# z430/keyword-spotting

Measured on AMD Instinct MI355X. Metric: 1s 16kHz clips/sec end-to-end (wav->label), higher is better.
Workload: dtype f32

## Files before the change

### keyword-spotting_amd/csrc/kws_dscnn.hip

```cpp
#include <type_traits>

#include "kws_internal.h"
#include "kws_mfcc_dev.h"
#include "kws_split_mfma.h"

namespace kws {
namespace {


#ifndef KWS_DSCNN_WAVES
#define KWS_DSCNN_WAVES 8
#endif
#ifndef KWS_X_DSCNN_STAMP_TID
#define KWS_X_DSCNN_STAMP_TID 0
#endif
constexpr int NW = KWS_DSCNN_WAVES;
constexpr int NT = NW * 64;
constexpr int TW = 30;

constexpr int P0 = C1_H * C1_W;
constexpr int FEAT_H = 103, FEAT_W = 14;
constexpr int OFF_Z3 = 0, OFF_Z2 = 22976, OFF_Z1 = 0, OFF_Z0 = 9152, OFF_FEAT = 18304;
constexpr int OFF_DWTAB = 38784;
constexpr int OFF_PWB = OFF_DWTAB + 2 * 768;
constexpr int OFF_POOLED = OFF_PWB + 2 * 64;
constexpr int OFF_POOLBUF = OFF_DWTAB;
constexpr int OFF_WMAX = OFF_POOLED + 64 + 8;
constexpr int LDS_FLOATS = 40960;
static_assert(OFF_WMAX + 4 * NW <= LDS_FLOATS, "LDS overflow");
static_assert(NW * 64 <= 768, "pool scratch must fit one depthwise buffer");
static_assert(OFF_FEAT + FEAT_H * FEAT_W <= OFF_Z2, "feature pad overlaps Z2");
static_assert(CH * 12 <= 2 * NT, "table staging assumes at most two elements per thread");

__device__ __forceinline__ constexpr int pidx(int c, int p, int S) { return (c >> 1) * 2 * S + 2 * p + (c & 1); }

template <int N>
struct Blk {
    static constexpr int H = 45 + 2 * N, W = 1 + 2 * N;
    static constexpr bool RING = N > 1;
    static constexpr int HI = RING ? H - 2 : H, WI = RING ? W - 2 : W;
    static constexpr int PIN = HI * WI, SIN = PIN + 2;
    static constexpr int POUT = H * W, SOUT = POUT + 2;
    static constexpr int OFF_IN = N == 1 ? OFF_Z0 : N == 2 ? OFF_Z1 : N == 3 ? OFF_Z2 : OFF_Z3;
    static constexpr int OFF_OUT = N == 1 ? OFF_Z1 : N == 2 ? OFF_Z2 : OFF_Z3;
    static constexpr int TILES = (POUT + TW - 1) / TW;
    static constexpr int BUF = (N - 1) & 1;
};

#ifndef KWS_DSCNN_KSPLIT_LEFTOVER
#define KWS_DSCNN_KSPLIT_LEFTOVER 1
#endif
template <int N>
struct Leftover {
    static constexpr bool HAS = KWS_DSCNN_KSPLIT_LEFTOVER && (N == 1 || N == 2);
    static constexpr int TILE = N == 1 ? 4 : 8;
    static constexpr int P0T = TILE * TW;
    static constexpr int NP = HAS ? Blk<N>::POUT - P0T : 1;
    static constexpr int WAVE0 = N == 1 ? 4 : 0;
    static constexpr int OFF_PART = N == 1 ? OFF_Z2 : OFF_Z0;
};
static_assert(Blk<1>::TILES == 5 && Blk<2>::TILES == 9, "the leftover tiles are the fifth of block 1 and the ninth of block 2");
static_assert(4 * CH * Leftover<1>::NP <= 38784 - OFF_Z2 && OFF_Z0 + 4 * CH * Leftover<2>::NP <= OFF_FEAT, "partial sums fit their dead planes");

constexpr int OFF_FEAT_P = OFF_Z2;
constexpr int OFF_POOLBUF_P = OFF_FEAT_P + 1456;
constexpr int STAGE_WAVES = 4;
static_assert(OFF_FEAT_P >= OFF_Z3 + Blk<3>::SOUT * CH, "the next clip's features must not overlap block 4's input");
static_assert(OFF_FEAT_P + FEAT_H * FEAT_W <= OFF_POOLBUF_P && OFF_POOLBUF_P % 4 == 0, "features and pool partials are disjoint");
static_assert(OFF_POOLBUF_P + NW * CH <= OFF_Z2 + Blk<2>::SOUT * CH && OFF_Z2 + Blk<2>::SOUT * CH <= OFF_DWTAB,
              "pool partials stay inside the Z2 plane, clear of the table buffers the next clip's block 1 rewrites");

template <bool TO_MFMA = false>
__device__ __forceinline__ float stencil3x3(float w0, float w1, float w2, float w3, float w4, float w5, float w6,
                                            float w7, float w8, float b, float up, float mid, float dn, float mask_l,
                                            float mask_r) {
    float c, to_right, to_left;
    asm("v_mul_f32 %1, %3, %13\n\t"
        "v_mul_f32 %2, %5, %13\n\t"
        "v_fma_f32 %0, %4, %13, %12\n\t"
        "v_fmac_f32 %1, %6, %14\n\t"
        "v_fmac_f32 %2, %8, %14\n\t"
        "v_fmac_f32 %0, %7, %14\n\t"
        "v_fmac_f32 %1, %9, %15\n\t"
        "v_fmac_f32 %2, %11, %15\n\t"
        "v_fmac_f32 %0, %10, %15\n\t"
        "v_fmac_f32_dpp %0, %1, %16 wave_shr:1 row_mask:0xf bank_mask:0xf bound_ctrl:1\n\t"
        "v_fmac_f32_dpp %0, %2, %17 wave_shl:1 row_mask:0xf bank_mask:0xf bound_ctrl:1"
        : "=&v"(c), "=&v"(to_right), "=&v"(to_left)
        : "v"(w0), "v"(w1), "v"(w2), "v"(w3), "v"(w4), "v"(w5), "v"(w6), "v"(w7), "v"(w8), "v"(b), "v"(up), "v"(mid),
          "v"(dn), "v"(mask_l), "v"(mask_r));
    if constexpr (TO_MFMA) asm volatile("s_nop 1" : "+v"(c));
    return c;
}
struct DwPair {
    float4 l[5];
};
template <bool TO_MFMA, int E>
__device__ __forceinline__ float stencil3x3_of_pair(const DwPair& w, float up, float mid, float dn, float mask_l, float mask_r) {
    if constexpr (E == 0)
        return stencil3x3<TO_MFMA>(w.l[0].x, w.l[0].z, w.l[1].x, w.l[1].z, w.l[2].x, w.l[2].z, w.l[3].x, w.l[3].z, w.l[4].x, w.l[4].z, up, mid, dn,
                                   mask_l, mask_r);
    else
        return stencil3x3<TO_MFMA>(w.l[0].y, w.l[0].w, w.l[1].y, w.l[1].w, w.l[2].y, w.l[2].w, w.l[3].y, w.l[3].w, w.l[4].y, w.l[4].w, up, mid, dn,
                                   mask_l, mask_r);
}
__device__ __forceinline__ float half_wave_sum_to_last_lane(float v) {
    v = dpp_shift_add<0x111, 0xf>(v);
    v = dpp_shift_add<0x112, 0xf>(v);
    v = dpp_shift_add<0x114, 0xf>(v);
    v = dpp_shift_add<0x118, 0xf>(v);
    v = dpp_shift_add<0x142, 0xa>(v);
    return v;
}

struct BlockTables {
    float d0, d1, b;
};
__device__ __forceinline__ void fetch_block_tables(const DscnnWeights& w, int n, int tid, BlockTables& r) {
    const float* src = w.dw_w + (n - 1) * CH * 12;
    r.d0 = tid < CH * 12 ? src[tid] : 0.f;
    r.d1 = NT + tid < CH * 12 ? src[NT + tid] : 0.f;
    r.b = tid < CH ? w.pw_b[(n - 1) * CH + tid] : 0.f;
}
__device__ __forceinline__ void store_block_tables(float* lds, int n, int tid, const BlockTables& r, float s_dwb = 1.f, float s_pwb = 1.f,
                                                   float s_dww = 1.f) {
    float* dwtab = lds + OFF_DWTAB + ((n - 1) & 1) * 768;
    if (tid < CH * 12) dwtab[tid] = r.d0 * ((tid % 24) >> 1 == 9 ? s_dwb : s_dww);
    if (NT + tid < CH * 12) dwtab[NT + tid] = r.d1 * (((NT + tid) % 24) >> 1 == 9 ? s_dwb : s_dww);
    if (tid < CH) lds[OFF_PWB + ((n - 1) & 1) * 64 + tid] = r.b * s_pwb;
}
struct PairCtx {
    float s_dww = 1.f;
    float s_dwb = 1.f;
    float s_pwb = 1.f;
    float inv_out = 1.f;
};
__device__ __forceinline__ void cap_units(int& ky, int& sg, int k_w, float bz) {
    sg = ky + k_w;
    const int eb = (int)((__builtin_bit_cast(uint32_t, bz) >> 23) & 0xffu) - 126;
    int limit = 100 - eb;
    limit = limit > 120 ? 120 : limit;
    if (sg > limit) {
        ky -= sg - limit;
        sg = limit;
    }
}
__device__ __forceinline__ void publish_wave_max(float* lds, int set, int wv, int lane, float mx) {
    auto step = [](float m, auto ctrl, auto row_mask) {
        return fmaxf(m, __builtin_bit_cast(float, __builtin_amdgcn_update_dpp(__builtin_bit_cast(int, m), __builtin_bit_cast(int, m), decltype(ctrl)::value,
                                                                              decltype(row_mask)::value, 0xf, false)));
    };
    mx = step(mx, std::integral_constant<int, 0x111>{}, std::integral_constant<int, 0xf>{});
    mx = step(mx, std::integral_constant<int, 0x112>{}, std::integral_constant<int, 0xf>{});
    mx = step(mx, std::integral_constant<int, 0x114>{}, std::integral_constant<int, 0xf>{});
    mx = step(mx, std::integral_constant<int, 0x118>{}, std::integral_constant<int, 0xf>{});
    mx = step(mx, std::integral_constant<int, 0x142>{}, std::integral_constant<int, 0xa>{});
    mx = step(mx, std::integral_constant<int, 0x143>{}, std::integral_constant<int, 0xc>{});
    if (lane == 63) lds[OFF_WMAX + set * NW + wv] = mx;
}
__device__ __forceinline__ float read_stage_max(const float* lds, int set0, int n_sets) {
    static_assert(NW % 4 == 0 && OFF_WMAX % 4 == 0, "the stage maxima are read as float4s");
    float m = 0.f;
    const float4* q = reinterpret_cast<const float4*>(lds + OFF_WMAX + set0 * NW);
    for (int i = 0; i < (NW / 4) * n_sets; ++i) {
        const float4 v = q[i];
        m = fmaxf(fmaxf(m, fmaxf(v.x, v.y)), fmaxf(v.z, v.w));
    }
    return m;
}

template <int NP>
struct PwRing {
    uintx4 ring[2][2][NP];
};
struct PwRegsF32 {
    float wa[2][32];
};
template <int MODE>
using PwOperands = std::conditional_t<(MODE >= 4), PwRing<(MODE == 5 ? 2 : 3)>, PwRegsF32>;
__device__ __forceinline__ void load_pointwise(const DscnnWeights& w, int n, int lane, PwRegsF32& o) {
    const float* pw = w.pw_w + (n - 1) * CH * CH + 8 * (lane >> 5) * CH + (lane & 31);
#pragma unroll
    for (int ct = 0; ct < 2; ++ct)
#pragma unroll
        for (int s = 0; s < 32; ++s) o.wa[ct][s] = pw[(16 * (s >> 3) + (s & 7)) * CH + ct * 32];
}
template <int NP>
__device__ __forceinline__ void load_afrag(const DscnnWeights& w, int n, int m, int lane, uintx4 (&f)[2][NP]) {
    const uintx4* src = reinterpret_cast<const uintx4*>(NP == 2 ? w.pw_pair : w.pw_split) + (size_t)(n - 1) * (2 * 4 * NP * 64) + lane;
#pragma unroll
    for (int ct = 0; ct < 2; ++ct)
#pragma unroll
        for (int p = 0; p < NP; ++p) f[ct][p] = src[((ct * 4 + m) * NP + p) * 64];
}
__device__ __forceinline__ void load_block_head(const DscnnWeights& w, int n, int lane, PwRegsF32& o) { load_pointwise(w, n, lane, o); }
template <int NP>
__device__ __forceinline__ void load_block_head(const DscnnWeights& w, int n, int lane, PwRing<NP>& o) { load_afrag(w, n, 0, lane, o.ring[0]); }

template <bool MFMA>
__device__ __forceinline__ void conv1_phase(const DscnnWeights& w, float* lds, int tid, const float (&a)[50]) {
    const float* featp = lds + OFF_FEAT;
    float* z0 = lds + OFF_Z0;
    if constexpr (MFMA) {
        const int lane = tid & 63, wv = tid >> 6, half = lane >> 5, col = lane & 31;
        const int ct = wv & 1;
        for (int u = wv; u < 10; u += NW) {
            const int pt = u >> 1;
            const int pos = pt * 32 + col;
            const int posc = pos < P0 ? pos : P0 - 1;
            const int oh = posc / C1_W, ow = posc % C1_W;
// ... 138 lines not shown
            __builtin_amdgcn_sched_barrier(0);
            product(5);
        }
        if (DUAL && kb + 2 < 7) {
            load_other(kb + 2);
            __builtin_amdgcn_sched_barrier(0);
        }
    }
    acc += acc2;
    occ += occ2;
    if (pos < p_hi) {
#pragma unroll
        for (int r = 0; r < 16; r += 2) {
            const int co = ct * 32 + row_of(r, half);
            const float v0 = relu(fmaf(w.c1_b[co], sig0, acc[r])), v1 = relu(fmaf(w.c1_b[co + 1], sig0, acc[r + 1]));
            *reinterpret_cast<float2*>(z0 + pidx(co, pos, P0 + 2)) = make_float2(v0, v1);
            if constexpr (PAIR) mx = fmaxf(mx, fmaxf(v0, v1));
            if (DUAL) {
                const int oo = (ct ^ 1) * 32 + row_of(r, half);
                const float u0 = relu(fmaf(w.c1_b[oo], sig0, occ[r])), u1 = relu(fmaf(w.c1_b[oo + 1], sig0, occ[r + 1]));
                *reinterpret_cast<float2*>(z0 + pidx(oo, pos, P0 + 2)) = make_float2(u0, u1);
                if constexpr (PAIR) mx = fmaxf(mx, fmaxf(u0, u1));
            }
        }
    }
}

constexpr int C1W_ROWS = FEAT_H;
constexpr int OFF_C1W8 = OFF_Z1;
constexpr int OFF_C1P2 = OFF_C1W8 + 2 * C1W_ROWS * 3 * 4;
static_assert(OFF_C1P2 + 2 * C1W_ROWS * 3 <= OFF_Z0, "conv1's operand windows live where block 1's output goes later");
static_assert(2 * (C1_W - 1) + 9 < FEAT_W && 2 * (C1_H - 1) + 9 < FEAT_H, "window reach inside the padded map");

__device__ __forceinline__ void conv1_build_windows(float* lds, int tid, float sx, int off_feat = OFF_FEAT) {
    const float* featp = lds + off_feat;
    uint32_t* w8 = reinterpret_cast<uint32_t*>(lds + OFF_C1W8);
    uint32_t* p2 = reinterpret_cast<uint32_t*>(lds + OFF_C1P2);
    for (int i = tid; i < C1W_ROWS * 3; i += NT) {
        const float* src = featp + (i / 3) * FEAT_W + 2 * (i % 3);
        const float y[8] = {src[0], src[1], src[2], src[3], src[4], src[5], src[6], src[7]};
        uintx4 hi, lo;
        split_pair8(y, sx, hi, lo);
        *reinterpret_cast<uintx4*>(w8 + i * 4) = hi;
        *reinterpret_cast<uintx4*>(w8 + (C1W_ROWS * 3 + i) * 4) = lo;
        uint32_t h, l;
        split_pair2(src[8], src[9], sx, h, l);
        p2[i] = h;
        p2[C1W_ROWS * 3 + i] = l;
    }
}

template <bool DUAL>
__device__ __forceinline__ void conv1_unit_pairwin(const DscnnWeights& w, const float* lds, float* z0, int ptile, int ct, int lane,
                                                   const uintx4 (&c1f)[7][2], int p_lo, int p_hi, float sig0, float& mx) {
    const int half = lane >> 5, col = lane & 31;
    const int pos = p_lo + ptile * 32 + col;
    const int posc = pos < p_hi ? pos : p_hi - 1;
    const int oh = posc / C1_W, ow = posc % C1_W;
    const int wi = (2 * oh + 5 * half) * 3 + ow;
    const uintx4* w8 = reinterpret_cast<const uintx4*>(lds + OFF_C1W8) + wi;
    const uint32_t* p2 = reinterpret_cast<const uint32_t*>(lds + OFF_C1P2) + wi;
    const floatx16 zero = {0, 0, 0, 0, 0, 0, 0, 0, 0, 0, 0, 0, 0, 0, 0, 0};
    floatx16 acc = zero, acc2 = zero, occ = zero, occ2 = zero;
    const uintx4* osrc = reinterpret_cast<const uintx4*>(w.c1_pair) + (size_t)(ct ^ 1) * (7 * 2 * 64) + lane;
    uintx4 of[DUAL ? 7 : 1][2];
    if (DUAL) {
#pragma unroll
        for (int kb = 0; kb < 7; ++kb) {
            of[kb][0] = osrc[(kb * 2 + 0) * 64];
            of[kb][1] = osrc[(kb * 2 + 1) * 64];
        }
    }
    float4 cb[4], ob[DUAL ? 4 : 1];
#pragma unroll
    for (int q = 0; q < 4; ++q) {
        cb[q] = *reinterpret_cast<const float4*>(w.c1_b + ct * 32 + 8 * q + 4 * half);
        if (DUAL) ob[DUAL ? q : 0] = *reinterpret_cast<const float4*>(w.c1_b + (ct ^ 1) * 32 + 8 * q + 4 * half);
    }
    uintx4 bq[3][2];
    auto b_load = [&](int kb, uintx4 (&d)[2]) {
        if (kb < 5) {
            d[0] = w8[kb * 3];
            d[1] = w8[kb * 3 + C1W_ROWS * 3];
        } else if (kb == 5) {
#pragma unroll
            for (int i = 0; i < 4; ++i) {
                d[0][i] = p2[i * 3];
                d[1][i] = p2[i * 3 + C1W_ROWS * 3];
            }
        } else {
            d[0] = uintx4{p2[4 * 3], 0u, 0u, 0u};
            d[1] = uintx4{p2[4 * 3 + C1W_ROWS * 3], 0u, 0u, 0u};
        }
    };
    b_load(0, bq[0]);
    b_load(1, bq[1]);
#pragma unroll
    for (int kb = 0; kb < 7; ++kb) {
        if (kb + 2 < 7) b_load(kb + 2, bq[(kb + 2) % 3]);
        const uintx4 &bh = bq[kb % 3][0], &bl = bq[kb % 3][1];
        acc2 = mfma_f16(c1f[kb][0], bl, acc2);
        if (DUAL) occ2 = mfma_f16(of[DUAL ? kb : 0][0], bl, occ2);
        acc = mfma_f16(c1f[kb][1], bh, acc);
        if (DUAL) occ = mfma_f16(of[DUAL ? kb : 0][1], bh, occ);
        acc2 = mfma_f16(c1f[kb][0], bh, acc2);
        if (DUAL) occ2 = mfma_f16(of[DUAL ? kb : 0][0], bh, occ2);
    }
    acc += acc2;
    occ += occ2;
    if (pos < p_hi) {
#pragma unroll
        for (int r = 0; r < 16; r += 2) {
            const int co = ct * 32 + row_of(r, half);
            const float4 b4 = cb[r >> 2];
            const float b0 = (r & 2) ? b4.z : b4.x, b1 = (r & 2) ? b4.w : b4.y;
            const float v0 = relu(fmaf(b0, sig0, acc[r])), v1 = relu(fmaf(b1, sig0, acc[r + 1]));
            *reinterpret_cast<float2*>(z0 + pidx(co, pos, P0 + 2)) = make_float2(v0, v1);
            mx = fmaxf(mx, fmaxf(v0, v1));
            if (DUAL) {
                const int oo = (ct ^ 1) * 32 + row_of(r, half);
                const float4 o4 = ob[DUAL ? (r >> 2) : 0];
                const float c0 = (r & 2) ? o4.z : o4.x, c1 = (r & 2) ? o4.w : o4.y;
                const float u0 = relu(fmaf(c0, sig0, occ[r])), u1 = relu(fmaf(c1, sig0, occ[r + 1]));
                *reinterpret_cast<float2*>(z0 + pidx(oo, pos, P0 + 2)) = make_float2(u0, u1);
                mx = fmaxf(mx, fmaxf(u0, u1));
            }
        }
    }
}

struct PosRange {
    int lo, hi;
};

template <bool RANGED, int NP>
__device__ __forceinline__ void conv1_phase_split(const DscnnWeights& w, float* lds, int tid, const uintx4 (&c1f)[7][NP],
                                                  PosRange rg, float sx = 1.f, float sig0 = 1.f, int off_feat = OFF_FEAT) {
    static_assert(P0 > 4 * 32 && P0 <= 5 * 32 && NW >= 6, "conv1 work split: four dual tiles + one tile in two halves");
    const float* featp = lds + off_feat;
    float* z0 = lds + OFF_Z0;
    const int lane = tid & 63, wv = tid >> 6;
    float mx = 0.f;
    if constexpr (NP == 2) {
        if constexpr (RANGED) {
            const int n_pt = (rg.hi - rg.lo + 31) / 32;
            for (int u = wv; u < 2 * n_pt; u += NW) conv1_unit_pairwin<false>(w, lds, z0, u >> 1, u & 1, lane, c1f, rg.lo, rg.hi, sig0, mx);
        } else if (wv < 4)
            conv1_unit_pairwin<true>(w, lds, z0, wv, wv & 1, lane, c1f, 0, P0, sig0, mx);
        else if (wv < 6)
            conv1_unit_pairwin<false>(w, lds, z0, 4, wv & 1, lane, c1f, 0, P0, sig0, mx);
    } else if constexpr (RANGED) {
        const int n_pt = (rg.hi - rg.lo + 31) / 32;
        for (int u = wv; u < 2 * n_pt; u += NW) conv1_unit_split<false, NP>(w, featp, z0, u >> 1, u & 1, lane, c1f, rg.lo, rg.hi, sx, sig0, mx);
    } else if (wv < 4)
        conv1_unit_split<true, NP>(w, featp, z0, wv, wv & 1, lane, c1f, 0, P0, sx, sig0, mx);
    else if (wv < 6)
        conv1_unit_split<false, NP>(w, featp, z0, 4, wv & 1, lane, c1f, 0, P0, sx, sig0, mx);
    if constexpr (NP == 2) publish_wave_max(lds, 1, wv, lane, mx);
    if (tid < CH) {
        z0[pidx(tid, P0, P0 + 2)] = 0.f;
        z0[pidx(tid, P0 + 1, P0 + 2)] = 0.f;
    }
}

template <int N, int NP>
__device__ __forceinline__ void leftover_partial_unit(float* lds, int lane, int M, const uintx4 (&af)[2][NP]) {
    using G = Blk<N>;
    using L = Leftover<N>;
    const int half = lane >> 5, col = lane & 31;
    const float* dwtab = lds + OFF_DWTAB + G::BUF * 768;
    const float4* dwt4 = reinterpret_cast<const float4*>(dwtab) + half * 24;
    const int pos = L::P0T - 1 + col;
    const bool valid = col >= 1 && col <= TW && pos < G::POUT;
    const int posc = pos < G::POUT ? pos : G::POUT - 1;
    const int h = posc / G::W, x = posc % G::W;
    const float mask_l = x > 0 ? 1.f : 0.f, mask_r = x < G::W - 1 ? 1.f : 0.f;
    int ta[3];
#pragma unroll
    for (int dh = -1; dh <= 1; ++dh) {
        const int o = G::RING ? 1 : 0;
        const int hh = h + dh - o, xx = x - o;
        const bool inside = (unsigned)hh < (unsigned)G::HI && (unsigned)xx < (unsigned)G::WI;
        const bool in_map = (unsigned)(h + dh) < (unsigned)G::H;
        const int a = inside ? hh * G::WI + xx : ((G::RING && in_map) ? G::PIN : G::PIN + 1);
        ta[dh + 1] = G::OFF_IN + pidx(half * 8, a, G::SIN);
    }
    float y[8];
#pragma unroll
    for (int j = 0; j < 8; j += 2) {
        const int cs = 16 * M + j;
        const int o = cs * G::SIN;
        const float2 up = *reinterpret_cast<const float2*>(lds + ta[0] + o);
        const float2 mid = *reinterpret_cast<const float2*>(lds + ta[1] + o);
        const float2 dn = *reinterpret_cast<const float2*>(lds + ta[2] + o);
        DwPair wp;
#pragma unroll
        for (int i = 0; i < 5; ++i) wp.l[i] = dwt4[(cs >> 1) * 6 + i];
        y[j] = stencil3x3_of_pair<false, 0>(wp, up.x, mid.x, dn.x, mask_l, mask_r);
        y[j + 1] = stencil3x3_of_pair<false, 1>(wp, up.y, mid.y, dn.y, mask_l, mask_r);
    }
    floatx16 acc0 = {0, 0, 0, 0, 0, 0, 0, 0, 0, 0, 0, 0, 0, 0, 0, 0}, acc1 = acc0;
    if constexpr (NP == 2) {
        uintx4 bh, bl;
// ... 419 lines not shown
                    "v_add_f32_dpp %7, %7, %7 row_bcast:15 row_mask:0xa bank_mask:0xf\n\t"
                    "v_add_f32_dpp %8, %8, %8 row_bcast:15 row_mask:0xa bank_mask:0xf\n\t"
                    "v_add_f32_dpp %9, %9, %9 row_bcast:15 row_mask:0xa bank_mask:0xf\n\t"
                    "v_add_f32_dpp %10, %10, %10 row_bcast:15 row_mask:0xa bank_mask:0xf\n\t"
                    "v_add_f32_dpp %11, %11, %11 row_bcast:15 row_mask:0xa bank_mask:0xf\n\t"
                    "v_add_f32_dpp %12, %12, %12 row_bcast:15 row_mask:0xa bank_mask:0xf\n\t"
                    "v_add_f32_dpp %13, %13, %13 row_bcast:15 row_mask:0xa bank_mask:0xf\n\t"
                    "v_add_f32_dpp %14, %14, %14 row_bcast:15 row_mask:0xa bank_mask:0xf\n\t"
                    "v_add_f32_dpp %15, %15, %15 row_bcast:15 row_mask:0xa bank_mask:0xf"
                    : "+v"(q[0]), "+v"(q[1]), "+v"(q[2]), "+v"(q[3]), "+v"(q[4]), "+v"(q[5]), "+v"(q[6]), "+v"(q[7]), "+v"(q[8]), "+v"(q[9]), "+v"(q[10]), "+v"(q[11]), "+v"(q[12]), "+v"(q[13]), "+v"(q[14]), "+v"(q[15]));
            }
            if (col == 31) {
#pragma unroll
                for (int k = 0; k < 32; ++k) poolbuf[wv * CH + (k >> 4) * 32 + row_of(k & 15, half)] = psum[k >> 4][k & 15] * pc.inv_out;
            }
        }
    }
    (void)bias4;
}

template <int NP>
__device__ __forceinline__ void load_conv1_frags(const DscnnWeights& w, int wv, int lane, uintx4 (&c1f)[7][NP]) {
    const uintx4* src = reinterpret_cast<const uintx4*>(NP == 2 ? w.c1_pair : w.c1_split) + (size_t)(wv & 1) * (7 * NP * 64) + lane;
#pragma unroll
    for (int kb = 0; kb < 7; ++kb)
#pragma unroll
        for (int p = 0; p < NP; ++p) c1f[kb][p] = src[(kb * NP + p) * 64];
}

__device__ __forceinline__ int wave_argmax_first(float v, int lane, int C) {
    float m = v;
    m = fmaxf(m, __builtin_bit_cast(float, __builtin_amdgcn_update_dpp(__builtin_bit_cast(int, m), __builtin_bit_cast(int, m), 0x111, 0xf, 0xf, false)));
    m = fmaxf(m, __builtin_bit_cast(float, __builtin_amdgcn_update_dpp(__builtin_bit_cast(int, m), __builtin_bit_cast(int, m), 0x112, 0xf, 0xf, false)));
    m = fmaxf(m, __builtin_bit_cast(float, __builtin_amdgcn_update_dpp(__builtin_bit_cast(int, m), __builtin_bit_cast(int, m), 0x114, 0xf, 0xf, false)));
    m = fmaxf(m, __builtin_bit_cast(float, __builtin_amdgcn_update_dpp(__builtin_bit_cast(int, m), __builtin_bit_cast(int, m), 0x118, 0xf, 0xf, false)));
    m = fmaxf(m, __builtin_bit_cast(float, __builtin_amdgcn_update_dpp(__builtin_bit_cast(int, m), __builtin_bit_cast(int, m), 0x142, 0xa, 0xf, false)));
    m = fmaxf(m, __builtin_bit_cast(float, __builtin_amdgcn_update_dpp(__builtin_bit_cast(int, m), __builtin_bit_cast(int, m), 0x143, 0xc, 0xf, false)));
    const float vmax = __builtin_bit_cast(float, __builtin_amdgcn_readlane(__builtin_bit_cast(int, m), 63));
    const unsigned long long holders = __ballot(lane < C && v == vmax);
    return holders ? __ffsll(holders) - 1 : 0;
}

__device__ __forceinline__ DscnnWeights weights_for_this_clip() {
#if defined(__HIP_DEVICE_COMPILE__)
    using KArg = const __attribute__((address_space(4))) DscnnWeights*;
    KArg p = (KArg)__builtin_amdgcn_kernarg_segment_ptr();
    asm volatile("" : "+s"(p));
    return *p;
#else
    return DscnnWeights{};
#endif
}

template <bool PAIR>
__device__ __forceinline__ void stage_features_persist(float* lds, const float* __restrict__ feat, int clip, int tid) {
    constexpr int ST = STAGE_WAVES * 64;
    constexpr int FV = (IN_T * IN_F + ST - 1) / ST;
    static_assert(2 * STAGE_WAVES == NW, "each staging wavefront zeroes the maximum slot of one other wavefront");
    const int lane = tid & 63, wv = tid >> 6;
    const float* f = feat + (size_t)clip * (IN_T * IN_F);
    float fv[FV];
#pragma unroll
    for (int k = 0; k < FV; ++k) {
        const int i = tid + k * ST;
        fv[k] = i < IN_T * IN_F ? f[i] : 0.f;
    }
    float* featp = lds + OFF_FEAT_P;
    for (int i = tid; i < FEAT_H * FEAT_W; i += ST) {
        const int r = i / FEAT_W - 2, c = i % FEAT_W - 2;
        if (!((unsigned)r < (unsigned)IN_T && (unsigned)c < (unsigned)IN_F)) featp[i] = 0.f;
    }
#pragma unroll
    for (int k = 0; k < FV; ++k) {
        const int i = tid + k * ST;
        if (i < IN_T * IN_F) featp[(i / IN_F + 2) * FEAT_W + (i % IN_F) + 2] = fv[k];
    }
    if constexpr (PAIR) {
        float m = 0.f;
#pragma unroll
        for (int k = 0; k < FV; ++k) m = fmaxf(m, fabsf(fv[k]));
        publish_wave_max(lds, 0, wv, lane, m);
        if (lane == 63) lds[OFF_WMAX + wv + STAGE_WAVES] = 0.f;
    }
}

__device__ __forceinline__ void pool_fc_wave(const DscnnWeights& w, const float* lds, int lane, int clip, float* __restrict__ logits,
                                             int32_t* __restrict__ label, float* __restrict__ a_pool) {
    const int C = w.num_classes;
    float4 fcw[CH / 4];
    float fcb = 0.f;
    const float4* wr = reinterpret_cast<const float4*>(w.fc_w + (lane < C ? lane : 0) * CH);
#pragma unroll
    for (int c = 0; c < CH / 4; ++c) fcw[c] = wr[c];
    if (lane < C) fcb = w.fc_b[lane];
    const float ring_b = w.pw_b[3 * CH + lane];
    constexpr float RING_N = 55.f * 11.f - 53.f * 9.f;
    float s = 0.f;
#pragma unroll
    for (int k = 0; k < NW; ++k) s += lds[OFF_POOLBUF_P + k * CH + lane];
    s = fmaf(RING_N, relu(ring_b), s) * (1.0f / (55.f * 11.f));
    if (a_pool) a_pool[lane] = s;
    float acc = fcb;
#pragma unroll
    for (int c = 0; c < CH / 4; ++c) {
        const float4 a4 = fcw[c];
        acc = fmaf(a4.x, __builtin_bit_cast(float, __builtin_amdgcn_readlane(__builtin_bit_cast(int, s), 4 * c + 0)), acc);
        acc = fmaf(a4.y, __builtin_bit_cast(float, __builtin_amdgcn_readlane(__builtin_bit_cast(int, s), 4 * c + 1)), acc);
        acc = fmaf(a4.z, __builtin_bit_cast(float, __builtin_amdgcn_readlane(__builtin_bit_cast(int, s), 4 * c + 2)), acc);
        acc = fmaf(a4.w, __builtin_bit_cast(float, __builtin_amdgcn_readlane(__builtin_bit_cast(int, s), 4 * c + 3)), acc);
    }
    if (lane < C) logits[(size_t)clip * C + lane] = acc;
    const int idx = wave_argmax_first(lane < C ? acc : -INFINITY, lane, C);
    if (label && lane == 0) label[clip] = idx;
}


template <int MODE, bool DIAG = true, bool PRECONV = false, bool STREAM = false, bool CLUSTER = false, bool PERSIST = false>
__global__ __launch_bounds__(NT) void kws_dscnn_fwd_kernel(DscnnWeights w_arg, const float* __restrict__ feat, int B,
                                                           float* __restrict__ logits, int32_t* __restrict__ label,
                                                           float* __restrict__ act_arg,
                                                           unsigned long long* __restrict__ stamps_arg,
                                                           const int* __restrict__ ring_hops, StreamPush sp) {
    static_assert(!STREAM || (MODE >= 4 && !DIAG && !PRECONV), "the fused push exists for the product paths only");
    static_assert(!PERSIST || ((MODE == 4 || MODE == 5) && !PRECONV && !STREAM), "persistent workgroups: batched product paths only");
    constexpr bool PAIR = MODE == 5;
    constexpr int NP = PAIR ? 2 : 3;
    BlockTables t1_pre{};
    static_assert(!CLUSTER || STREAM, "time-tile clusters exist for the streaming push only");
    float* const act = DIAG ? act_arg : nullptr;
    unsigned long long* const stamps = DIAG ? stamps_arg : nullptr;
    extern __shared__ __attribute__((aligned(16))) float lds[];
    constexpr bool MFMA = MODE != 0;
    const int tid_k = threadIdx.x;
    const int lane_k = tid_k & 63, wv_k = tid_k >> 6;

    const int cl_n = CLUSTER ? sp.cluster : 1;
    int clip = CLUSTER ? (int)blockIdx.x / cl_n : (int)blockIdx.x;
    const int cl_tile = CLUSTER ? (int)blockIdx.x - clip * cl_n : 0;
    if (clip >= B) return;
    const int j0 = Blk<4>::H * cl_tile / cl_n, j1 = Blk<4>::H * (cl_tile + 1) / cl_n;
    auto rows = [&](int lo, int hi, int H, int W) { return PosRange{(lo < 0 ? 0 : lo) * W, (hi > H ? H : hi) * W}; };
    const PosRange rg4 = rows(j0, j1, Blk<4>::H, Blk<4>::W), rg3 = rows(j0 - 2, j1, Blk<3>::H, Blk<3>::W),
                   rg2 = rows(j0 - 4, j1, Blk<2>::H, Blk<2>::W), rg1 = rows(j0 - 6, j1, Blk<1>::H, Blk<1>::W),
                   rg0 = rows(j0 - 7, j1 + 1, C1_H, C1_W);
    int n_stamp = 0;
    auto stamp = [&]() {
        if (stamps && tid_k == KWS_X_DSCNN_STAMP_TID) stamps[(size_t)clip * KWS_DSCNN_STAMPS + n_stamp] = __builtin_amdgcn_s_memtime();
        ++n_stamp;
    };

    constexpr bool SPLIT = MODE >= 4;
    BlockTables t1p{};
    uintx4 c1p[PERSIST ? 7 : 1][NP];
    int prev_clip = -1;
    float* a_prev = nullptr;
    if constexpr (PERSIST) {
        fetch_block_tables(w_arg, 1, tid_k, t1p);
        if (wv_k < STAGE_WAVES) stage_features_persist<PAIR>(lds, feat, clip, tid_k);
        load_conv1_frags(w_arg, wv_k, lane_k, c1p);
        __syncthreads();
    }
    for (;;) {
    const DscnnWeights w = PERSIST ? weights_for_this_clip() : w_arg;
    int tid = tid_k;
    if constexpr (PERSIST) {
        int wv_l = __builtin_amdgcn_readfirstlane(wv_k), lane_l = lane_k;
        asm volatile("" : "+s"(wv_l), "+v"(lane_l));
        tid = (wv_l << 6) | (lane_l & 63);
    }
    const int lane = tid & 63, wv = tid >> 6;
    if constexpr (PERSIST) n_stamp = 0;
    if (stamps && tid == KWS_X_DSCNN_STAMP_TID) stamps[(size_t)clip * KWS_DSCNN_STAMPS + KWS_DSCNN_STAMPS - 2] = __builtin_amdgcn_s_memrealtime();
    stamp();

    PwOperands<MODE> wa;
    int hops_before = 0;
    int kx = 0, ky[5] = {0, 0, 0, 0, 0}, sg[5] = {0, 0, 0, 0, 0};
    if constexpr (PERSIST) {
        if constexpr (PAIR) {
            const float mxf = read_stage_max(lds, 0, 1);
            kx = pow2_exp_for(mxf);
            const float bz0 = (w.c1_abs * mxf + w.c1_bmax) * 1.001f;
            cap_units(kx, sg[0], w.k_c1, bz0);
            const float by1 = (w.dw_abs[0] * bz0 + w.dw_bmax[0]) * 1.001f;
            ky[1] = pow2_exp_for(by1);
            cap_units(ky[1], sg[1], w.k_pw[0], (w.pw_abs[0] * by1 + w.pw_bmax[0]) * 1.001f);
            store_block_tables(lds, 1, tid, t1p, pow2f(ky[1]), pow2f(sg[1]), pow2f(ky[1] - sg[0]));
            conv1_build_windows(lds, tid, pow2f(kx), OFF_FEAT_P);
            __syncthreads();
        } else {
            store_block_tables(lds, 1, tid, t1p);
        }
        stamp();
        conv1_phase_split<false, NP>(w, lds, tid, c1p, rg0, pow2f(kx), pow2f(sg[0]), OFF_FEAT_P);
        if (wv == NW - 1 && prev_clip >= 0) {
            pool_fc_wave(w, lds, lane, prev_clip, logits, label, a_prev);
            if (stamps && lane == 0) stamps[(size_t)prev_clip * KWS_DSCNN_STAMPS + 13] = __builtin_amdgcn_s_memtime();
        }
        load_afrag(w, 1, wv >= 4 ? wv - 4 : 0, lane, wa.ring[0]);
    } else if constexpr (PRECONV) {
        static_assert(!PRECONV || MODE >= 4, "the pre-convolved entry exists for the product (split) path only");
        const float* z = feat + (size_t)clip * (CH * P0);
        fetch_block_tables(w, 1, tid, t1_pre);
        float zmax = 0.f;
        for (int i = tid; i < CH * P0; i += NT) {
            const float v = z[i];
            lds[OFF_Z0 + pidx(i / P0, i % P0, P0 + 2)] = v;
            zmax = fmaxf(zmax, v);
        }
        if (tid < CH) {
            lds[OFF_Z0 + pidx(tid, P0, P0 + 2)] = 0.f;
            lds[OFF_Z0 + pidx(tid, P0 + 1, P0 + 2)] = 0.f;
        }
        if constexpr (PAIR)
            publish_wave_max(lds, 1, wv, lane, zmax);
        else
            store_block_tables(lds, 1, tid, t1_pre);
        if constexpr (Leftover<1>::HAS && (MODE == 4 || MODE == 5) && !CLUSTER)
            load_afrag(w, 1, wv >= 4 ? wv - 4 : 0, lane, wa.ring[0]);
        else
            load_block_head(w, 1, lane, wa);
        stamp();
    } else {
    float* featp = lds + OFF_FEAT;
    const float* f = feat + (size_t)clip * (IN_T * IN_F);
    constexpr int FV = (IN_T * IN_F + NT - 1) / NT;
    float fv[FV];
    int row_new = -1;
    int head;
    if constexpr (STREAM) {
        hops_before = *sp.hops;
        const int K = (sp.p.frame_len + sp.p.frame_step - 1) / sp.p.frame_step;
        head = (((hops_before + 2 - K) % IN_T) + IN_T) % IN_T;
        const int step = sp.p.frame_step;
        const long f_start = (long)step * hops_before + step - (long)((sp.p.frame_len + step - 1) / step) * step;
        if (f_start >= 0) row_new = (int)((((f_start / step) - head) % IN_T + IN_T) % IN_T);
    } else {
        head = ring_hops ? (((*ring_hops + 1 - sp.frames_lag) % IN_T) + IN_T) % IN_T : 0;
    }
#pragma unroll
    for (int k = 0; k < FV; ++k) {
        const int i = tid + k * NT;
        fv[k] = (i < IN_T * IN_F && i / IN_F != row_new) ? f[((i / IN_F + head) % IN_T) * IN_F + i % IN_F] : 0.f;
    }
    BlockTables t1;
    fetch_block_tables(w, 1, tid, t1);
    __builtin_amdgcn_sched_barrier(0);
// ... 121 lines not shown
    if constexpr (PAIR) {
        const float mz = fmaxf(read_stage_max(lds, 2, (Leftover<1>::HAS && KSL_ON) ? 2 : 1) * pow2f(-sg[1]), w.pw_bmax[0]);
        const float bz = (w.pw_abs[1] * ((w.dw_abs[1] * mz + w.dw_bmax[1]) * 1.001f) + w.pw_bmax[1]) * 1.001f;
        const float by = (w.dw_abs[2] * bz + w.dw_bmax[2]) * 1.001f;
        ky[3] = pow2_exp_for(by);
        cap_units(ky[3], sg[3], w.k_pw[2], (w.pw_abs[2] * by + w.pw_bmax[2]) * 1.001f);
        pc.s_dww = pow2f(ky[3] - sg[2]);
        pc.s_dwb = pow2f(ky[3]);
        pc.s_pwb = pow2f(sg[3]);
    }
    block_phase<2, MODE, CLUSTER>(w, lds, tid, wa, nullptr, rg2, pc);
    stamp();
    __syncthreads();
    if constexpr (Leftover<2>::HAS && KSL_ON) {
        leftover_combine<2, PAIR>(lds, tid);
        __syncthreads();
    }
    stamp();
    if (a) {
        const float u = PAIR ? pow2f(-sg[2]) : 1.f;
        for (int i = tid; i < CH * Blk<2>::POUT; i += NT)
            a[i] = lds[OFF_Z2 + pidx(i / Blk<2>::POUT, i % Blk<2>::POUT, Blk<2>::SOUT)] * u;
        a += CH * Blk<2>::POUT;
    }
    if constexpr (PAIR) {
        const float mz = fmaxf(read_stage_max(lds, 0, (Leftover<2>::HAS && KSL_ON) ? 2 : 1) * pow2f(-sg[2]), w.pw_bmax[1]);
        const float bz = (w.pw_abs[2] * ((w.dw_abs[2] * mz + w.dw_bmax[2]) * 1.001f) + w.pw_bmax[2]) * 1.001f;
        const float by = (w.dw_abs[3] * bz + w.dw_bmax[3]) * 1.001f;
        ky[4] = pow2_exp_for(by);
        cap_units(ky[4], sg[4], w.k_pw[3], (w.pw_abs[3] * by + w.pw_bmax[3]) * 1.001f);
        pc.s_dww = pow2f(ky[4] - sg[3]);
        pc.s_dwb = pow2f(ky[4]);
        pc.s_pwb = pow2f(sg[4]);
    }
    block_phase<3, MODE, CLUSTER>(w, lds, tid, wa, nullptr, rg3, pc);
    stamp();
    __syncthreads();
    stamp();
    if (a) {
        const float u = PAIR ? pow2f(-sg[3]) : 1.f;
        for (int i = tid; i < CH * Blk<3>::POUT; i += NT)
            a[i] = lds[OFF_Z3 + pidx(i / Blk<3>::POUT, i % Blk<3>::POUT, Blk<3>::SOUT)] * u;
        a += CH * Blk<3>::POUT;
    }
    if constexpr (PAIR) {
        pc.inv_out = pow2f(-sg[4]);
    }
    block_phase<4, MODE, CLUSTER>(w, lds, tid, wa, a ? a + CH : nullptr, rg4, pc,
                                  PERSIST ? OFF_POOLBUF_P : OFF_POOLBUF);
    stamp();
    if constexpr (PERSIST) {
        const int next = clip + (int)gridDim.x;
        __builtin_amdgcn_sched_barrier(0);
        if (wv < STAGE_WAVES && next < B) stage_features_persist<PAIR>(lds, feat, next, tid);
        stamp();
        load_conv1_frags(w, wv, lane, c1p);
        __syncthreads();
        stamp();
        if (stamps && tid == KWS_X_DSCNN_STAMP_TID) stamps[(size_t)clip * KWS_DSCNN_STAMPS + KWS_DSCNN_STAMPS - 1] = __builtin_amdgcn_s_memrealtime();
        prev_clip = clip;
        a_prev = a;
        clip = next;
        if (clip >= B) break;
        continue;
    }
    const int C = w.num_classes;
    float4 fcw[CH / 4];
    float fcb = 0.f, ring_b = 0.f;
    if (wv == 0 && lane < C) {
        const float4* wr = reinterpret_cast<const float4*>(w.fc_w + lane * CH);
#pragma unroll
        for (int c = 0; c < CH / 4; ++c) fcw[c] = wr[c];
        fcb = w.fc_b[lane];
    }
    if (tid < CH) ring_b = w.pw_b[3 * CH + tid];
    __syncthreads();
    stamp();

    float* pooled = lds + OFF_POOLED;
    constexpr float RING_N = 55.f * 11.f - 53.f * 9.f;
    bool run_fc = true;
    if constexpr (CLUSTER) {
        float* part = sp.cl_part + ((size_t)clip * cl_n + cl_tile) * CH;
        if (tid < CH) {
            float s = 0.f;
#pragma unroll
            for (int k = 0; k < NW; ++k) s += lds[OFF_POOLBUF + k * CH + tid];
            __hip_atomic_store(part + tid, s, __ATOMIC_RELAXED, __HIP_MEMORY_SCOPE_AGENT);
        }
        asm volatile("s_waitcnt vmcnt(0)" ::: "memory");
        __syncthreads();
        int* last_flag = reinterpret_cast<int*>(lds + OFF_POOLED + CH);
        if (tid == 0) {
            const int arrived = atomicAdd(&sp.cl_count[clip], 1);
            *last_flag = arrived == cl_n - 1;
            if (arrived == cl_n - 1) sp.cl_count[clip] = 0;
        }
        __syncthreads();
        run_fc = *last_flag != 0;
        if (run_fc) {
            if (tid < CH) {
                float s = 0.f;
                for (int t = 0; t < cl_n; ++t)
                    s += __hip_atomic_load(sp.cl_part + ((size_t)clip * cl_n + t) * CH + tid, __ATOMIC_RELAXED, __HIP_MEMORY_SCOPE_AGENT);
                pooled[tid] = fmaf(RING_N, relu(ring_b), s) * (1.0f / (55.f * 11.f));
            }
        }
// ... 326 lines not shown
```

Measured before the change: 7.062 million.

## Build conv1 split windows during next-clip staging to drop a barrier

Result: no change. 7.111 million (median of 6 runs) (+0.7%).

```diff
diff --git a/keyword-spotting_amd/csrc/kws_dscnn.hip b/keyword-spotting_amd/csrc/kws_dscnn.hip
--- a/keyword-spotting_amd/csrc/kws_dscnn.hip
+++ b/keyword-spotting_amd/csrc/kws_dscnn.hip
@@ -64,11 +64,18 @@
 
 constexpr int OFF_FEAT_P = OFF_Z2;
 constexpr int OFF_POOLBUF_P = OFF_FEAT_P + 1456;
+constexpr int OFF_C1W_P = OFF_POOLBUF_P + NW * CH;
+constexpr int C1W_FLOATS = 2 * FEAT_H * 3 * 4 + 2 * FEAT_H * 3;
 constexpr int STAGE_WAVES = 4;
+constexpr int STAGE_ROWS = (FEAT_H + STAGE_WAVES - 1) / STAGE_WAVES;
 static_assert(OFF_FEAT_P >= OFF_Z3 + Blk<3>::SOUT * CH, "the next clip's features must not overlap block 4's input");
 static_assert(OFF_FEAT_P + FEAT_H * FEAT_W <= OFF_POOLBUF_P && OFF_POOLBUF_P % 4 == 0, "features and pool partials are disjoint");
 static_assert(OFF_POOLBUF_P + NW * CH <= OFF_Z2 + Blk<2>::SOUT * CH && OFF_Z2 + Blk<2>::SOUT * CH <= OFF_DWTAB,
               "pool partials stay inside the Z2 plane, clear of the table buffers the next clip's block 1 rewrites");
+static_assert(OFF_C1W_P == OFF_POOLBUF_P + NW * CH && OFF_C1W_P % 4 == 0, "the windows follow the pool partials, 16-byte aligned");
+static_assert(OFF_C1W_P + C1W_FLOATS <= OFF_Z2 + 4 * CH * Leftover<1>::NP && OFF_Z2 + 4 * CH * Leftover<1>::NP <= OFF_Z2 + Blk<2>::SOUT * CH,
+              "the windows end inside the stretch block 1's leftover partials take: written behind conv1's barrier, when the windows are dead");
+static_assert(STAGE_ROWS <= 64 && STAGE_ROWS * STAGE_WAVES >= FEAT_H, "one lane per padded row of a staging wavefront's share");
 
 template <bool TO_MFMA = false>
 __device__ __forceinline__ float stencil3x3(float w0, float w1, float w2, float w3, float w4, float w5, float w6,
@@ -145,7 +152,7 @@
         sg = limit;
     }
 }
-__device__ __forceinline__ void publish_wave_max(float* lds, int set, int wv, int lane, float mx) {
+__device__ __forceinline__ float wave_max_to_last_lane(float mx) {
     auto step = [](float m, auto ctrl, auto row_mask) {
         return fmaxf(m, __builtin_bit_cast(float, __builtin_amdgcn_update_dpp(__builtin_bit_cast(int, m), __builtin_bit_cast(int, m), decltype(ctrl)::value,
                                                                               decltype(row_mask)::value, 0xf, false)));
@@ -156,6 +163,10 @@
     mx = step(mx, std::integral_constant<int, 0x118>{}, std::integral_constant<int, 0xf>{});
     mx = step(mx, std::integral_constant<int, 0x142>{}, std::integral_constant<int, 0xa>{});
     mx = step(mx, std::integral_constant<int, 0x143>{}, std::integral_constant<int, 0xc>{});
+    return mx;
+}
+__device__ __forceinline__ void publish_wave_max(float* lds, int set, int wv, int lane, float mx) {
+    mx = wave_max_to_last_lane(mx);
     if (lane == 63) lds[OFF_WMAX + set * NW + wv] = mx;
 }
 __device__ __forceinline__ float read_stage_max(const float* lds, int set0, int n_sets) {
@@ -400,14 +411,15 @@
 
 template <bool DUAL>
 __device__ __forceinline__ void conv1_unit_pairwin(const DscnnWeights& w, const float* lds, float* z0, int ptile, int ct, int lane,
-                                                   const uintx4 (&c1f)[7][2], int p_lo, int p_hi, float sig0, float& mx) {
+                                                   const uintx4 (&c1f)[7][2], int p_lo, int p_hi, float sig0, float& mx,
+                                                   int off_win = OFF_C1W8) {
     const int half = lane >> 5, col = lane & 31;
     const int pos = p_lo + ptile * 32 + col;
     const int posc = pos < p_hi ? pos : p_hi - 1;
     const int oh = posc / C1_W, ow = posc % C1_W;
     const int wi = (2 * oh + 5 * half) * 3 + ow;
-    const uintx4* w8 = reinterpret_cast<const uintx4*>(lds + OFF_C1W8) + wi;
-    const uint32_t* p2 = reinterpret_cast<const uint32_t*>(lds + OFF_C1P2) + wi;
+    const uintx4* w8 = reinterpret_cast<const uintx4*>(lds + off_win) + wi;
+    const uint32_t* p2 = reinterpret_cast<const uint32_t*>(lds + off_win + (OFF_C1P2 - OFF_C1W8)) + wi;
     const floatx16 zero = {0, 0, 0, 0, 0, 0, 0, 0, 0, 0, 0, 0, 0, 0, 0, 0};
     floatx16 acc = zero, acc2 = zero, occ = zero, occ2 = zero;
     const uintx4* osrc = reinterpret_cast<const uintx4*>(w.c1_pair) + (size_t)(ct ^ 1) * (7 * 2 * 64) + lane;
@@ -483,7 +495,8 @@
 
 template <bool RANGED, int NP>
 __device__ __forceinline__ void conv1_phase_split(const DscnnWeights& w, float* lds, int tid, const uintx4 (&c1f)[7][NP],
-                                                  PosRange rg, float sx = 1.f, float sig0 = 1.f, int off_feat = OFF_FEAT) {
+                                                  PosRange rg, float sx = 1.f, float sig0 = 1.f, int off_feat = OFF_FEAT,
+                                                  int off_win = OFF_C1W8) {
     static_assert(P0 > 4 * 32 && P0 <= 5 * 32 && NW >= 6, "conv1 work split: four dual tiles + one tile in two halves");
     const float* featp = lds + off_feat;
     float* z0 = lds + OFF_Z0;
@@ -492,11 +505,11 @@
     if constexpr (NP == 2) {
         if constexpr (RANGED) {
             const int n_pt = (rg.hi - rg.lo + 31) / 32;
-            for (int u = wv; u < 2 * n_pt; u += NW) conv1_unit_pairwin<false>(w, lds, z0, u >> 1, u & 1, lane, c1f, rg.lo, rg.hi, sig0, mx);
+            for (int u = wv; u < 2 * n_pt; u += NW) conv1_unit_pairwin<false>(w, lds, z0, u >> 1, u & 1, lane, c1f, rg.lo, rg.hi, sig0, mx, off_win);
         } else if (wv < 4)
-            conv1_unit_pairwin<true>(w, lds, z0, wv, wv & 1, lane, c1f, 0, P0, sig0, mx);
+            conv1_unit_pairwin<true>(w, lds, z0, wv, wv & 1, lane, c1f, 0, P0, sig0, mx, off_win);
         else if (wv < 6)
-            conv1_unit_pairwin<false>(w, lds, z0, 4, wv & 1, lane, c1f, 0, P0, sig0, mx);
+            conv1_unit_pairwin<false>(w, lds, z0, 4, wv & 1, lane, c1f, 0, P0, sig0, mx, off_win);
     } else if constexpr (RANGED) {
         const int n_pt = (rg.hi - rg.lo + 31) / 32;
         for (int u = wv; u < 2 * n_pt; u += NW) conv1_unit_split<false, NP>(w, featp, z0, u >> 1, u & 1, lane, c1f, rg.lo, rg.hi, sx, sig0, mx);
@@ -1022,12 +1035,9 @@
 #endif
 }
 
-template <bool PAIR>
 __device__ __forceinline__ void stage_features_persist(float* lds, const float* __restrict__ feat, int clip, int tid) {
     constexpr int ST = STAGE_WAVES * 64;
     constexpr int FV = (IN_T * IN_F + ST - 1) / ST;
-    static_assert(2 * STAGE_WAVES == NW, "each staging wavefront zeroes the maximum slot of one other wavefront");
-    const int lane = tid & 63, wv = tid >> 6;
     const float* f = feat + (size_t)clip * (IN_T * IN_F);
     float fv[FV];
 #pragma unroll
@@ -1045,12 +1055,67 @@
         const int i = tid + k * ST;
         if (i < IN_T * IN_F) featp[(i / IN_F + 2) * FEAT_W + (i % IN_F) + 2] = fv[k];
     }
-    if constexpr (PAIR) {
-        float m = 0.f;
-#pragma unroll
-        for (int k = 0; k < FV; ++k) m = fmaxf(m, fabsf(fv[k]));
-        publish_wave_max(lds, 0, wv, lane, m);
-        if (lane == 63) lds[OFF_WMAX + wv + STAGE_WAVES] = 0.f;
+}
+
+__device__ __forceinline__ void stage_operands_persist(const DscnnWeights& w, float* lds, const float* __restrict__ feat, int clip, int wv,
+                                                       int lane) {
+    static_assert(2 * STAGE_WAVES == NW, "each staging wavefront zeroes the maximum slot of one other wavefront");
+    static_assert(IN_F == 10 && FEAT_W == IN_F + 4 && FEAT_H == IN_T + 4 && IN_T > 64 && IN_T <= 128 && (IN_T * IN_F) % 2 == 0,
+                  "a lane holds whole feature rows as five 8-byte loads; two loads per lane cover the clip");
+    const float* f = feat + (size_t)clip * (IN_T * IN_F);
+    const int own = STAGE_ROWS * wv - 2 + lane;
+    int r1 = own < 0 ? own + IN_T : own;
+    r1 = r1 >= IN_T ? r1 - IN_T : r1;
+    const bool has2 = lane < IN_T - 64;
+    int r2 = own + 64;
+    r2 = r2 >= IN_T ? r2 - IN_T : r2;
+    r2 = has2 ? r2 : 0;
+    float2 fa[IN_F / 2], fb[IN_F / 2];
+#pragma unroll
+    for (int j = 0; j < IN_F / 2; ++j) fa[j] = reinterpret_cast<const float2*>(f + r1 * IN_F)[j];
+#pragma unroll
+    for (int j = 0; j < IN_F / 2; ++j) fb[j] = has2 ? reinterpret_cast<const float2*>(f + r2 * IN_F)[j] : make_float2(0.f, 0.f);
+    float m = 0.f;
+#pragma unroll
+    for (int j = 0; j < IN_F / 2; ++j) {
+        m = fmaxf(m, fmaxf(fabsf(fa[j].x), fabsf(fa[j].y)));
+        m = fmaxf(m, fmaxf(fabsf(fb[j].x), fabsf(fb[j].y)));
+    }
+    m = wave_max_to_last_lane(m);
+    const float mxf = __builtin_bit_cast(float, __builtin_amdgcn_readlane(__builtin_bit_cast(int, m), 63));
+    int kx = pow2_exp_for(mxf), sg0;
+    const float bz0 = (w.c1_abs * mxf + w.c1_bmax) * 1.001f;
+    cap_units(kx, sg0, w.k_c1, bz0);
+    const float sx = pow2f(kx);
+    const int row = STAGE_ROWS * wv + lane;
+    if (lane < STAGE_ROWS && row < FEAT_H) {
+        const bool live = (unsigned)own < (unsigned)IN_T;
+        float pr[FEAT_W];
+        pr[0] = pr[1] = pr[FEAT_W - 2] = pr[FEAT_W - 1] = 0.f;
+#pragma unroll
+        for (int j = 0; j < IN_F / 2; ++j) {
+            pr[2 + 2 * j] = live ? fa[j].x : 0.f;
+            pr[3 + 2 * j] = live ? fa[j].y : 0.f;
+        }
+        uint32_t* w8 = reinterpret_cast<uint32_t*>(lds + OFF_C1W_P);
+        uint32_t* p2 = w8 + 2 * C1W_ROWS * 3 * 4;
+#pragma unroll
+        for (int s = 0; s < 3; ++s) {
+            const int i = row * 3 + s;
+            const float y[8] = {pr[2 * s], pr[2 * s + 1], pr[2 * s + 2], pr[2 * s + 3], pr[2 * s + 4], pr[2 * s + 5], pr[2 * s + 6], pr[2 * s + 7]};
+            uintx4 hi, lo;
+            split_pair8(y, sx, hi, lo);
+            *reinterpret_cast<uintx4*>(w8 + i * 4) = hi;
+            *reinterpret_cast<uintx4*>(w8 + (C1W_ROWS * 3 + i) * 4) = lo;
+            uint32_t h, l;
+            split_pair2(pr[2 * s + 8], pr[2 * s + 9], sx, h, l);
+            p2[i] = h;
+            p2[C1W_ROWS * 3 + i] = l;
+        }
+    }
+    if (lane == 63) {
+        lds[OFF_WMAX + wv] = mxf;
+        lds[OFF_WMAX + wv + STAGE_WAVES] = 0.f;
     }
 }
 
@@ -1126,7 +1191,12 @@
     float* a_prev = nullptr;
     if constexpr (PERSIST) {
         fetch_block_tables(w_arg, 1, tid_k, t1p);
-        if (wv_k < STAGE_WAVES) stage_features_persist<PAIR>(lds, feat, clip, tid_k);
+        if (wv_k < STAGE_WAVES) {
+            if constexpr (PAIR)
+                stage_operands_persist(w_arg, lds, feat, clip, __builtin_amdgcn_readfirstlane(wv_k), lane_k);
+            else
+                stage_features_persist(lds, feat, clip, tid_k);
+        }
         load_conv1_frags(w_arg, wv_k, lane_k, c1p);
         __syncthreads();
     }
@@ -1156,13 +1226,11 @@
             ky[1] = pow2_exp_for(by1);
             cap_units(ky[1], sg[1], w.k_pw[0], (w.pw_abs[0] * by1 + w.pw_bmax[0]) * 1.001f);
             store_block_tables(lds, 1, tid, t1p, pow2f(ky[1]), pow2f(sg[1]), pow2f(ky[1] - sg[0]));
-            conv1_build_windows(lds, tid, pow2f(kx), OFF_FEAT_P);
-            __syncthreads();
         } else {
             store_block_tables(lds, 1, tid, t1p);
         }
         stamp();
-        conv1_phase_split<false, NP>(w, lds, tid, c1p, rg0, pow2f(kx), pow2f(sg[0]), OFF_FEAT_P);
+        conv1_phase_split<false, NP>(w, lds, tid, c1p, rg0, pow2f(kx), pow2f(sg[0]), OFF_FEAT_P, OFF_C1W_P);
         if (wv == NW - 1 && prev_clip >= 0) {
             pool_fc_wave(w, lds, lane, prev_clip, logits, label, a_prev);
             if (stamps && lane == 0) stamps[(size_t)prev_clip * KWS_DSCNN_STAMPS + 13] = __builtin_amdgcn_s_memtime();
@@ -1390,7 +1458,12 @@
     if constexpr (PERSIST) {
         const int next = clip + (int)gridDim.x;
         __builtin_amdgcn_sched_barrier(0);
-        if (wv < STAGE_WAVES && next < B) stage_features_persist<PAIR>(lds, feat, next, tid);
+        if (wv < STAGE_WAVES && next < B) {
+            if constexpr (PAIR)
+                stage_operands_persist(w, lds, feat, next, wv, lane);
+            else
+                stage_features_persist(lds, feat, next, tid);
+        }
         stamp();
         load_conv1_frags(w, wv, lane, c1p);
         __syncthreads();
```
